# danisotelo/qm_door

Measured on AMD Instinct MI355X. Metric: MPC+WBC cycles/sec (AlienGo+Z1, N=100), higher is better.
Workload: dtype f64

## Files before the change

### qm_door_amd/csrc/kernels/aux_kernels.h

```cpp
#pragma once
#include "layout.h"
#include "lq_kernel.h"

namespace qmk {

__global__ void __launch_bounds__(64) input_weight_kernel(const ProblemR* P, const real* zeros, real* Rw) {
  __shared__ real J[12 * 12];
  __shared__ real RJ[12 * 12];
  const int lane = threadIdx.x;
  const ModelR& md = P->model;
  const int dd = lane < AD_DIRS ? lane : AD_DIRS - 1;
  const AdIn in{P->settings.initial_state, zeros, P->settings.initial_state, dd, 0.0_r};
  FlowOut<Du, Du3, Du3> f;
  BaseMotion2<Du, Du3> bm;
  centroidalSweep2<Du, Du3, Du3>(
      md, P->settings.gravity, in,
      [&](int c, Vec3<Du>, Vec3<Du3> v) {
        if (lane >= 3 && lane < 15) { const int j = lane - 3; J[(3 * c + 0) * 12 + j] = v.x.e; J[(3 * c + 1) * 12 + j] = v.y.e; J[(3 * c + 2) * 12 + j] = v.z.e; }
      },
      [&](Vec3<Du>, const Mat3<Du>&) { return Vec3<Du3>(); }, f, bm);
  __syncthreads();
  const real* Rt = P->settings.R_task;
  for (int e = lane; e < 144; e += 64) {
    const int i = e / 12, j = e % 12;
    real s = 0.0_r;
    for (int k = 0; k < 12; ++k) s += Rt[(12 + i) * 30 + 12 + k] * J[k * 12 + j];
    RJ[e] = s;
  }
  __syncthreads();
  for (int e = lane; e < 900; e += 64) {
    const int i = e / 30, j = e % 30;
    real v = Rt[e];
    if (i >= 12 && i < 24 && j >= 12 && j < 24) {
      v = 0.0_r;
// ... 102 lines not shown
      const real len = tb[q] - ta[q];
      const real a = (len > 2.0_r * REAL_EPS) ? (tb[q] - t[q]) / len : 1.0_r;
      const bool before = interval < 0 || K <= 1, after = !before && interval >= last;
      idx[q] = before ? 0 : (after ? max(last - 1, 0) : interval);
      alpha[q] = before ? 1.0_r : (after ? 0.0_r : a);
    }
    const bool isX = lane < 30, isU = lane >= 32 && lane < 62;
    const int c = isX ? lane : (isU ? lane - 32 : 0);
    real l[NB], r[NB];
#pragma unroll
    for (int q = 0; q < NB; ++q) {
      const int iu0 = min(idx[q], Np - 1), iu1 = min(idx[q] + 1, Np - 1);
      const real* pl = isU ? Up + (size_t(inst) * Np + iu0) * 30 : Xp + (size_t(inst) * (Np + 1) + idx[q]) * 30;
      const real* pr = isU ? Up + (size_t(inst) * Np + iu1) * 30 : Xp + (size_t(inst) * (Np + 1) + min(idx[q] + 1, last)) * 30;
      l[q] = pl[c]; r[q] = pr[c];
    }
    const real x0v = (x0 && isX) ? x0[size_t(inst) * 30 + c] : 0.0_r;
#pragma unroll
    for (int q = 0; q < NB; ++q) { QM_KEEP(l[q]); QM_KEEP(r[q]); }
#pragma unroll
    for (int q = 0; q < NB; ++q) {
      const int k = k0 + q;
      const real v = alpha[q] * l[q] + (1.0_r - alpha[q]) * r[q];
      if (k <= Nn && isX) warmX[(size_t(inst) * (Nn + 1) + k) * 30 + c] = (k == 0 && x0) ? x0v : v;
      else if (k < Nn && isU) warmU[(size_t(inst) * Nn + k) * 30 + c] = v;
    }
  }
}

__global__ void __launch_bounds__(64) policy_eval_kernel(int batch, int N, const real* tgrid, const real* X, const real* U, const int* modes, const real* tEval,
                                                         real* xOut, real* uOut, int* modeOut) {
  const int inst = blockIdx.x, lane = threadIdx.x;
  if (inst >= batch) return;
  const real* tg = tgrid + size_t(inst) * (N + 1);
  const real t = tEval[inst];
  int idx; real alpha;
  timeSegmentWave(tg, N + 1, t, lane, idx, alpha);
  const int kMode = gridCountBelow(tg + 1, N, t, lane);
  if (lane < 30) {
    const real* xl = X + (size_t(inst) * (N + 1) + idx) * 30;
    xOut[size_t(inst) * 30 + lane] = alpha * xl[lane] + (1.0_r - alpha) * xl[30 + lane];
  } else if (lane >= 32 && lane < 62) {
    const int i = lane - 32, iu0 = min(idx, N - 1), iu1 = min(idx + 1, N - 1);
    const real* ul = U + (size_t(inst) * N + iu0) * 30; const real* ur = U + (size_t(inst) * N + iu1) * 30;
    uOut[size_t(inst) * 30 + i] = alpha * ul[i] + (1.0_r - alpha) * ur[i];
  } else if (lane == 63) {
    modeOut[inst] = modes[size_t(inst) * (N + 1) + kMode];
  }
}

}
```

### qm_door_amd/csrc/kernels/gpu_rt.h

```cpp
#pragma once
#ifdef QMGPU_HOST_EMULATION
#include "real.h"
#include "simt_emu.h"
#else
#include <hip/hip_runtime.h>
#include "real.h"
namespace qmk {
#ifdef QM_WAVE_SYNC_BARE
#define QM_WAVE_SYNC() __builtin_amdgcn_wave_barrier()
#else
#define QM_WAVE_SYNC() do { __builtin_amdgcn_fence(__ATOMIC_RELEASE, "wavefront"); __builtin_amdgcn_wave_barrier(); __builtin_amdgcn_fence(__ATOMIC_ACQUIRE, "wavefront"); } while (0)
#endif
__device__ __forceinline__ double qmFromWords(int lo, int hi, double) { return __hiloint2double(hi, lo); }
__device__ __forceinline__ float qmFromWords(int lo, int, float) { return __int_as_float(lo); }
__device__ __forceinline__ int qmLoWord(double v) { return __double2loint(v); }
__device__ __forceinline__ int qmHiWord(double v) { return __double2hiint(v); }
__device__ __forceinline__ int qmLoWord(float v) { return __float_as_int(v); }
__device__ __forceinline__ int qmHiWord(float) { return 0; }
__device__ __forceinline__ real qmShflXor(real v, int mask) { return __shfl_xor(v, mask, 64); }
__device__ __forceinline__ real qmReadLane(real v, int src) {
  const int lo = __builtin_amdgcn_readlane(qmLoWord(v), src);
  const int hi = sizeof(real) == 8 ? __builtin_amdgcn_readlane(qmHiWord(v), src) : 0;
  return qmFromWords(lo, hi, real());
}
__device__ __forceinline__ int qmReadLaneInt(int v, int src) { return __builtin_amdgcn_readlane(v, src); }
__device__ __forceinline__ unsigned long long qmBallot(bool p) { return __builtin_amdgcn_ballot_w64(p); }
__device__ __forceinline__ int qmFirstBit(unsigned long long m) { return __builtin_ctzll(m); }
__device__ __forceinline__ int qmPopCount(unsigned long long m) { return __builtin_popcountll(m); }
typedef double QmAccD __attribute__((ext_vector_type(4)));
typedef float QmAccF __attribute__((ext_vector_type(4)));
template <class T> struct QmAccOf { typedef QmAccD type; };
template <> struct QmAccOf<float> { typedef QmAccF type; };
typedef QmAccOf<real>::type QmAcc;
typedef real QmD2 __attribute__((ext_vector_type(2)));
__device__ __forceinline__ void qmMfma(QmAccD& c, double a, double b) { c = __builtin_amdgcn_mfma_f64_16x16x4f64(a, b, c, 0, 0, 0); }
__device__ __forceinline__ void qmMfma(QmAccF& c, float a, float b) { c = __builtin_amdgcn_mfma_f32_16x16x4f32(a, b, c, 0, 0, 0); }
__device__ __forceinline__ constexpr int qmARow(int p) { return sizeof(real) == 8 ? p : (p >> 2) + 4 * (p & 3); }
__device__ __forceinline__ double qmMulNoFma(double a, double b) { return __dmul_rn(a, b); }
__device__ __forceinline__ double qmSubNoFma(double a, double b) { return __dsub_rn(a, b); }
__device__ __forceinline__ double qmRsqrtPos(double x) {
  const double y = __builtin_amdgcn_rsq(x);
  const double e = __builtin_fma(-x * y, y, 1.0);
  return __builtin_fma(y * e, __builtin_fma(e, 0.375, 0.5), y);
}
__device__ __forceinline__ float qmRsqrtPos(float x) { return __builtin_amdgcn_rsqf(x); }
__device__ __forceinline__ double qmRcpPos(double x) {
  double y = __builtin_amdgcn_rcp(x);
  y = __builtin_fma(y, __builtin_fma(-x, y, 1.0), y);
  return __builtin_fma(y, __builtin_fma(-x, y, 1.0), y);
}
__device__ __forceinline__ float qmRcpPos(float x) { return __builtin_amdgcn_rcpf(x); }
template <int R, bool FIRST> __device__ __forceinline__ void qmFmacRowBcast(double& acc, double bc, double m) {
  if (FIRST) asm volatile("s_nop 1\n\tv_fmac_f64_dpp %0, %1, %2 row_newbcast:%3 row_mask:0xf bank_mask:0xf" : "+v"(acc) : "v"(bc), "v"(m), "n"(R));
  else asm volatile("v_fmac_f64_dpp %0, %1, %2 row_newbcast:%3 row_mask:0xf bank_mask:0xf" : "+v"(acc) : "v"(bc), "v"(m), "n"(R));
}
template <int R, bool FIRST> __device__ __forceinline__ void qmFmacRowBcast(float& acc, float bc, float m) {
  if (FIRST) asm volatile("s_nop 1\n\tv_fmac_f32_dpp %0, %1, %2 row_newbcast:%3 row_mask:0xf bank_mask:0xf" : "+v"(acc) : "v"(bc), "v"(m), "n"(R));
  else asm volatile("v_fmac_f32_dpp %0, %1, %2 row_newbcast:%3 row_mask:0xf bank_mask:0xf" : "+v"(acc) : "v"(bc), "v"(m), "n"(R));
}
template <int G> __device__ __forceinline__ real qmReplicateRow(real v) {
  const int addr = (16 * G + (int(threadIdx.x) & 15)) * 4;
  const int lo = __builtin_amdgcn_ds_bpermute(addr, qmLoWord(v));
  const int hi = sizeof(real) == 8 ? __builtin_amdgcn_ds_bpermute(addr, qmHiWord(v)) : 0;
  return qmFromWords(lo, hi, real());
}
__device__ __forceinline__ real qmReplicateRow0(real v) { return qmReplicateRow<0>(v); }
#define QM_TO_LDS_PTR(T, p) ((const T __attribute__((address_space(3)))*)(p))
template <class T> __device__ __forceinline__ const T* qmConstantPtr(const T* p) {
  const T __attribute__((address_space(4)))* p4 = (const T __attribute__((address_space(4)))*)(p);
  asm("" : "+s"(p4));
  return (const T*)p4;
}
// ... 62 lines not shown
```

### qm_door_amd/csrc/kernels/linesearch_kernel.h

```cpp
#pragma once
#include "layout.h"
#include "ls_lds.h"
#include "schedule_dev.h"
#include "sweep_dev.h"

namespace qmk {

struct LsArgs {
  const ProblemR* P;
  const real* Rw;
  int batch, N, K, lineSearch;
  const real* eeContact;
  const real* tgrid; const real* dtgrid; const int* nodePhase;
  const real* X; const real* U; const real* dX; const real* dU;
  const real* targetTimes; const real* targetStates;
  const int* schedNum; const real* schedTimes; const int* schedModes;
  const real* metrics;
  const real* instStats;
  const int* nodeMode;
  real* Xt; real* Ut;
  real* outT; real* outX; real* outU; int* outMode; real* outStats;
  int iteration;
  int trialInLds;
  int* done;
};

inline int lsThreads(int B, int N, int cus) { return (B > cus && N + 1 <= LS_MAX_THREADS / 2) ? LS_MAX_THREADS / 2 : LS_MAX_THREADS; }
struct LsLaunch { int threads, dynamicLdsBytes, trialInLds; };
inline LsLaunch lsLaunch(int B, int N, int cus) {
  const int threads = lsThreads(B, N, cus), bytes = lsTrialLdsBytes(N, threads);
  return LsLaunch{threads, bytes, bytes > 0};
}

struct DblIn {
  const real* x; const real* u; real dtS; const real* k1;
  __device__ __forceinline__ real hn(int i) const { return x[i] + dtS * k1[i]; }
  __device__ __forceinline__ real euler(int i) const { return x[9 + i] + dtS * k1[9 + i]; }
  __device__ __forceinline__ real q(int j) const { return x[12 + j] + dtS * u[12 + j]; }
  __device__ __forceinline__ real qd(int j) const { return u[12 + j]; }
  __device__ __forceinline__ Vec3<real> force(int c) const { return Vec3<real>(u[3 * c], u[3 * c + 1], u[3 * c + 2]); }
};

template <class WP> __device__ __attribute__((noinline)) void nodePerformance(const ModelR& md, const SettingsR& st, WP Qw, WP Rw, int weightStructure, const real* bc, const Schedule& sched, const real* tTimes, const real* tStates, const real* contact, int K, real t, real dt, int phase,
                                       bool terminal, const real* x, const real* u, const real* xnext, real& cost, real& dyn, real& eq, real* xnOut = nullptr) {
  QM_TICK_DECL;
  const int mode = sched.modes[phase];
  real eePosRef[3], eeQuatRef[4];
  eeReference(tTimes, tStates, K, t, eePosRef, eeQuatRef);
  real Ke = 0.0_r, fRef[3] = {0.0_r, 0.0_r, 0.0_r}, pEnv[3] = {0.0_r, 0.0_r, 0.0_r};
  if (contact && !terminal) { Ke = st.ee_contact_stiffness; eeContactReference(tTimes, contact, K, t, fRef, pEnv); }
  real k1[12];
#pragma unroll
  for (int i = 0; i < 12; ++i) k1[i] = 0.0_r;
  real c = 0.0_r;
  dyn = 0.0_r; eq = 0.0_r;
  real phi[12];
#pragma unroll 1
// ... 110 lines not shown
}
__device__ __forceinline__ real sumSquaresStrided(const real* v, int n, int first, int stride) {
  constexpr int UN = 8;
  real s = 0.0_r;
  for (int base = first; base < n; base += UN * stride) {
    real t[UN];
#pragma unroll
    for (int q = 0; q < UN; ++q) { const int e = base + q * stride; t[q] = v[e < n ? e : first]; }
#pragma unroll
    for (int q = 0; q < UN; ++q) QM_KEEP(t[q]);
#pragma unroll
    for (int q = 0; q < UN; ++q) { const int e = base + q * stride; if (e < n) s += t[q] * t[q]; }
  }
  return s;
}

#ifdef QM_RICCATI_TIMING
#define QM_LS_CLOCK(slot) do { const unsigned long long n_ = clock64(); if (blockIdx.x == 0 && threadIdx.x == 0) qmk::qmRiccatiTicks[240 + (slot)] += n_ - lsClk; lsClk = n_; } while (0)
#else
#define QM_LS_CLOCK(slot)
#endif
#if defined(QM_LS_EXTERN) && !defined(QM_RICCATI_TIMING)
__global__ void __launch_bounds__(LS_MAX_THREADS) linesearch_kernel(LsArgs a);
#else
__global__ void __launch_bounds__(LS_MAX_THREADS) linesearch_kernel(LsArgs a) {
#ifdef QM_RICCATI_TIMING
  unsigned long long lsClk = clock64();
#endif
  __shared__ LsRed red; __shared__ LsCtlWords ctl; __shared__ LsVotes structVotes; __shared__ ModelR mdS;
  __shared__ __attribute__((aligned(16))) LsWeights wQ, wR;
  static_assert(lsLdsBytes(sizeof(red)) + lsLdsBytes(sizeof(ctl)) + lsLdsBytes(sizeof(structVotes)) + lsLdsBytes(sizeof(mdS)) + lsLdsBytes(sizeof(wQ)) + lsLdsBytes(sizeof(wR)) == LS_STATIC_LDS_BYTES,
                "a __shared__ array added here goes into this sum and into LS_STATIC_LDS_BYTES by hand: compare both with .group_segment_fixed_size in the assembly");
  const int inst = blockIdx.x, tid = threadIdx.x, nthr = blockDim.x;
  if (a.done[inst]) return;
  const int N = a.N;
  const SettingsR& st = a.P->settings;
  const real* tg = a.tgrid + size_t(inst) * (N + 1);
  const Schedule sched{a.schedNum[inst], a.schedTimes + size_t(inst) * QMGPU_MAX_EVENTS, a.schedModes + size_t(inst) * (QMGPU_MAX_EVENTS + 1)};
  const real* tTimes = a.targetTimes + size_t(inst) * a.K;
  const real* tStates = a.targetStates + size_t(inst) * a.K * QMGPU_NTARGET;
  const real* X = a.X + size_t(inst) * (N + 1) * 30; const real* U = a.U + size_t(inst) * N * 30;
  const real* dX = a.dX + size_t(inst) * (N + 1) * 30; const real* dU = a.dU + size_t(inst) * N * 30;
  const int half = (N + 1 <= nthr / 2) ? nthr / 2 : nthr;
  const int nTr = nthr / half, myTr = tid / half, ltid = tid - myTr * half;
  QM_DYNAMIC_LDS(trialLds);
  real* Xt = a.trialInLds ? trialLds + size_t(myTr) * lsTrialRows(N) * NX : a.Xt + (size_t(inst) * 2 + myTr) * (N + 1) * 30;
  real* Ut = a.trialInLds ? Xt + (N + 1) * NX : a.Ut + (size_t(inst) * 2 + myTr) * N * 30;

  constexpr int MDW = (int(sizeof(ModelR) / 4) + LS_MAX_THREADS - 1) / LS_MAX_THREADS;
  int mdw[2 * MDW];
  const int mdPer = nthr >= LS_MAX_THREADS ? MDW : 2 * MDW;
  real m0 = 0.0_r, d0 = 0.0_r, e0 = 0.0_r;
  {
    bool outside = false;
    real qv[4], rv4[4];
#pragma unroll
    for (int q4 = 0; q4 < 4; ++q4) { const int e = tid + q4 * nthr, ec = e < 900 ? e : tid; qv[q4] = st.Q[ec]; rv4[q4] = a.Rw[ec]; }
    {
      const int* src = reinterpret_cast<const int*>(&a.P->model);
#pragma unroll
      for (int w = 0; w < 2 * MDW; ++w) { const int e = tid + w * nthr; mdw[w] = (w < mdPer && e < int(sizeof(ModelR) / 4)) ? src[e] : 0; }
    }
    real mk[3] = {0.0_r, 0.0_r, 0.0_r};
    if (tid <= N) { const real* m = a.metrics + (size_t(inst) * (N + 1) + tid) * NODE_METRICS; mk[0] = m[0]; mk[1] = m[1]; mk[2] = m[2]; }
#pragma unroll
    for (int q4 = 0; q4 < 4; ++q4) { QM_KEEP(qv[q4]); QM_KEEP(rv4[q4]); }
#pragma unroll
    for (int w = 0; w < 2 * MDW; ++w) QM_KEEP(mdw[w]);
// ... 69 lines not shown
        const real al = tr ? alpha * st.alpha_decay : alpha;
        if (tr && al < st.alpha_min) break;
        real s0 = 0, s1 = 0, s2 = 0;
        const int nTrial = N + 1 < half ? N + 1 : half;
        for (int i = tr * half; i < tr * half + nTrial; ++i) { s0 += red[0][i]; s1 += red[1][i]; s2 += red[2][i]; }
        m1 = s0; v1 = sqrt(s1 + s2);
        bool ok;
        if (!a.lineSearch) { ok = true; type = 0; }
        else if (v1 > st.g_max) { ok = v1 < (1.0_r - st.gamma_c) * viol0; type = 1; }
        else if (v1 < st.g_min && viol0 < st.g_min && al * armijo < 0.0_r) { ok = m1 < merit0 + st.armijo_factor * al * armijo; type = 3; }
        else { ok = m1 < merit0 - st.gamma_c * viol0 || v1 < (1.0_r - st.gamma_c) * viol0; type = 2; }
        accAlpha = al;
        if (ok) acc = 1.0_r;
      }
      ctl[LS_MERIT1] = m1; ctl[LS_VIOL1] = v1; ctl[LS_ACCEPTED] = acc; ctl[LS_STEP_TYPE] = real(type); ctl[LS_ALPHA] = accAlpha;
    }
    __syncthreads();
    QM_LS_CLOCK(4);
    merit1 = ctl[LS_MERIT1]; viol1 = ctl[LS_VIOL1]; stepType = int(ctl[LS_STEP_TYPE]);
    accepted = ctl[LS_ACCEPTED] != 0.0_r;
    const real lastAlpha = ctl[LS_ALPHA];
    __syncthreads();
    if (accepted) { alpha = lastAlpha; break; }
    alpha = lastAlpha * st.alpha_decay;
    if (alpha < st.alpha_min) break;
  }
  if (!accepted) { alpha = 0.0_r; stepType = 4; merit1 = merit0; viol1 = viol0; }
  real* oX = a.outX + size_t(inst) * (N + 1) * 30; real* oU = a.outU + size_t(inst) * N * 30;
  axpyStrided(oX, X, dX, alpha, (N + 1) * 30, tid, nthr);
  axpyStrided(oU, U, dU, alpha, N * 30, tid, nthr);
  for (int k = tid; k <= N; k += nthr) { a.outT[size_t(inst) * (N + 1) + k] = tg[k]; a.outMode[size_t(inst) * (N + 1) + k] = a.nodeMode[size_t(inst) * (N + 1) + k]; }
  QM_LS_CLOCK(5);
  const real sx = sumSquaresStrided(dX, (N + 1) * 30, tid, nthr), su = sumSquaresStrided(dU, N * 30, tid, nthr);
  __syncthreads();
  red[0][tid] = sx; red[1][tid] = su;
  __syncthreads();
  if (tid == 0) {
    real s0 = 0, s1 = 0;
    for (int i = 0; i < nthr; ++i) { s0 += red[0][i]; s1 += red[1][i]; }
    int conv = 0;
    if (a.iteration + 1 >= st.sqp_iterations) conv = 1;
    else if (alpha < st.alpha_min) conv = 2;
    else if (fabs(merit1 - merit0) < st.cost_tol && viol1 < st.g_min) conv = 3;
    else if (alpha * sqrt(s0) < st.delta_tol && alpha * sqrt(s1) < st.delta_tol) conv = 4;
    if (ricStatus != 0.0_r && conv == 0) conv = 2;
    a.done[inst] = conv;
    if (a.outStats) {
      real* s = a.outStats + size_t(inst) * QMGPU_NSTATS;
      s[0] = merit0; s[1] = viol0; s[2] = merit1; s[3] = viol1; s[4] = alpha; s[5] = real(stepType); s[6] = armijo; s[7] = ricStatus;
      s[8] = real(a.iteration + 1); s[9] = real(conv);
    }
  }
  QM_LS_CLOCK(6);
}
#endif

}
```

### qm_door_amd/csrc/kernels/mpc_pipeline.h

```cpp
#pragma once
#include <vector>

#include "../host/host_error.h"
#include "aux_kernels.h"
#include "ddp_kernel.h"
#include "gpu_rt.h"
#include "layout.h"
#include "linesearch_kernel.h"
#include "lq_kernel.h"
#include "riccati_kernel.h"

namespace qmk {

struct MpcBuffers {
  ProblemR* dP = nullptr;
  real *dRw = nullptr, *dZeros = nullptr;
  real *dTgrid = nullptr, *dDtgrid = nullptr, *dX = nullptr, *dU = nullptr, *dStages = nullptr, *dAdRows = nullptr, *dMetrics = nullptr, *dGains = nullptr, *ddX = nullptr, *ddU = nullptr;
  real *dXt = nullptr, *dUt = nullptr, *dInstStats = nullptr, *dDebug = nullptr;
  int *dStageNc = nullptr, *dNodeMode = nullptr, *dNodePhase = nullptr, *dDone = nullptr;
  real *dDdpX = nullptr, *dDdpU = nullptr, *dDdpMerit = nullptr;
  int cus = 256;
  size_t maxBatch = 0, maxNodes = 0;
};

struct MpcIo {
  int batch, N, K, lineSearch;
  double dtD;
  const double *t0D, *timeGridD, *schedTimesD;
  const real *x0, *targetTimes, *targetStates;
  const int* schedNum; const real* schedTimes; const int* schedModes;
  const real *warmX, *warmU;
  real *outT, *outX, *outU; int* outMode; real* outStats;
  const real* eeContact;
  int algorithm;
};

template <class Alloc> inline void allocateMpcBuffers(MpcBuffers& m, size_t B, size_t N, Alloc&& alloc) {
  const size_t N1 = N + 1;
  m.maxBatch = B; m.maxNodes = N;
  auto R = [&](size_t n, bool scratch = true) { return static_cast<real*>(alloc(n, sizeof(real), scratch)); };
  auto I = [&](size_t n) { return static_cast<int*>(alloc(n, sizeof(int), true)); };
  m.dP = static_cast<ProblemR*>(alloc(1, sizeof(ProblemR), false));
  m.dRw = R(QM_RW_DOUBLES, false);
  m.dZeros = R(64, false);
  m.dTgrid = R(B * N1);
  m.dDtgrid = R(B * N1);
  m.dNodePhase = I(B * N1);
  m.dX = R(B * N1 * 30);
  m.dU = R(B * N * 30);
  m.dStages = R(B * N1 * STAGE_DOUBLES);
  m.dAdRows = R(B * N1 * AD_DOUBLES);
  m.dMetrics = R(B * N1 * NODE_METRICS);
  m.dGains = R(B * N * GAIN_DOUBLES);
  m.ddX = R(B * N1 * 30);
  m.ddU = R(B * N * 30);
  m.dXt = R(2 * B * N1 * 30);
  m.dUt = R(2 * B * N * 30);
  m.dInstStats = R(B * 4);
  m.dStageNc = I(B * N1);
  m.dNodeMode = I(B * N1);
  m.dDone = I(B);
  int dev = 0, cus = 0;
  if (hipGetDevice(&dev) == hipSuccess && hipDeviceGetAttribute(&cus, hipDeviceAttributeMultiprocessorCount, dev) == hipSuccess && cus > 0) m.cus = cus;
}

template <class Alloc> inline void ensureDdpBuffers(MpcBuffers& m, Alloc&& alloc) {
  if (m.dDdpX) return;
  const size_t B = m.maxBatch, N = m.maxNodes;
// ... 25 lines not shown
  io.warmX = in(a.warm_x, st.warmX, B * N1 * 30);
  io.warmU = in(a.warm_u, st.warmU, B * N * 30);
  io.eeContact = in(a.ee_contact_ref, st.eeContact, B * K * 6);
  io.outT = outT; io.outX = outX; io.outU = outU; io.outMode = a.out_mode; io.outStats = outStats;
  io.algorithm = a.algorithm;
  return io;
}

enum TimingEvent { EV_START, EV_AD_NODE, EV_LQ_NODE, EV_RICCATI, EV_LINE_SEARCH, EV_WBC_START, EV_WBC_END, TIMING_EVENTS = EV_WBC_END + 1 };
inline void recordTiming(hipEvent_t* ev, TimingEvent which, hipStream_t s) { if (ev) (void)hipEventRecord(ev[which], s); }

inline void enqueueLqRiccati(hipStream_t s, const MpcBuffers& m, const MpcIo& io, real* debug, hipEvent_t* ev) {
  const int B = io.batch, N = io.N;
  LqArgs la{m.dP, m.dRw, B, N, io.K, m.dTgrid, m.dDtgrid, m.dNodePhase, m.dX, m.dU, io.targetTimes, io.targetStates, io.schedNum, io.schedTimes,
            io.schedModes, m.dZeros, m.dStages, m.dStageNc, m.dNodeMode, m.dMetrics, debug, m.dAdRows, m.dDone, io.eeContact};
  QM_LAUNCH(ad_node_kernel, adGridFor(B * (N + 1)), 64, s, la);
  recordTiming(ev, EV_AD_NODE, s);
  QM_LAUNCH(lq_node_kernel, B * (N + 1), 64, s, la);
  recordTiming(ev, EV_LQ_NODE, s);
  RiccatiArgs ra{B, N, m.dStages, m.dStageNc, m.dDtgrid, io.x0, m.dX, m.dGains, m.ddX, m.ddU, m.dInstStats, m.dDone};
  QM_LAUNCH_DYN(riccati_kernel<RICCATI_WAVES>, B, RICCATI_WAVES * 64, RICCATI_LDS_BYTES, s, ra);
  recordTiming(ev, EV_RICCATI, s);
}

inline void enqueueMpcKernels(hipStream_t s, const MpcBuffers& m, const MpcIo& io, int iterations, bool debugLq, hipEvent_t* ev) {
  const int B = io.batch, N = io.N;
  recordTiming(ev, EV_START, s);
  for (int it = 0; it < iterations; ++it) {
    InitArgs ia{m.dP, B, N, io.dtD, io.t0D, io.timeGridD, io.schedTimesD, io.x0, it == 0 ? io.warmX : io.outX, it == 0 ? io.warmU : io.outU, io.schedNum, io.schedModes,
                m.dTgrid, m.dDtgrid, m.dNodePhase, m.dX, m.dU, it, m.dDone};
    QM_LAUNCH(mpc_init_kernel, B, 128, s, ia);
    enqueueLqRiccati(s, m, io, debugLq ? m.dDebug : nullptr, ev);
    const LsLaunch shape = lsLaunch(B, N, m.cus);
    LsArgs ls{m.dP, m.dRw, B, N, io.K, io.lineSearch, io.eeContact, m.dTgrid, m.dDtgrid, m.dNodePhase, m.dX, m.dU, m.ddX, m.ddU, io.targetTimes, io.targetStates, io.schedNum,
              io.schedTimes, io.schedModes, m.dMetrics, m.dInstStats, m.dNodeMode, m.dXt, m.dUt, io.outT, io.outX, io.outU, io.outMode, io.outStats, it, shape.trialInLds, m.dDone};
    QM_LAUNCH_DYN(linesearch_kernel, B, shape.threads, shape.dynamicLdsBytes, s, ls);
    recordTiming(ev, EV_LINE_SEARCH, s);
  }
}

inline void enqueueDdpKernels(hipStream_t s, const MpcBuffers& m, const MpcIo& io, int trials, hipEvent_t* ev) {
  const int B = io.batch, N = io.N;
  recordTiming(ev, EV_START, s);
  InitArgs ia{m.dP, B, N, io.dtD, io.t0D, io.timeGridD, io.schedTimesD, io.x0, io.warmX, io.warmU, io.schedNum, io.schedModes, m.dTgrid, m.dDtgrid, m.dNodePhase, m.dX, m.dU, 0, m.dDone};
  QM_LAUNCH(mpc_init_kernel, B, 128, s, ia);
  DdpArgs ra{m.dP, m.dRw, B, N, io.K, 0, io.eeContact, m.dTgrid, m.dDtgrid, m.dNodePhase, io.x0, m.dX, m.dU, io.targetTimes, io.targetStates, io.schedNum, io.schedTimes, io.schedModes,
             m.dStages, m.dStageNc, m.dGains, m.dX, m.dU, m.dDdpMerit};
  if (!io.warmX) QM_LAUNCH(ddp_rollout_kernel, (B + 63) / 64, 64, s, ra);
  enqueueLqRiccati(s, m, io, nullptr, ev);
  ra.trials = trials; ra.Xout = m.dDdpX; ra.Uout = m.dDdpU;
  QM_LAUNCH(ddp_rollout_kernel, (B * trials + 63) / 64, 64, s, ra);
  DdpSelectArgs sa{m.dP, B, N, trials, m.dTgrid, m.dNodeMode, m.dX, m.dU, m.dMetrics, m.dInstStats, m.dDdpX, m.dDdpU, m.dDdpMerit, io.outT, io.outX, io.outU, io.outMode, io.outStats, m.dDone};
  QM_LAUNCH(ddp_select_kernel, B, 256, s, sa);
  recordTiming(ev, EV_LINE_SEARCH, s);
}

inline int ddpTrialCount(double minStep, double maxStep) {
  int n = 0;
  for (double a = maxStep; a >= minStep && n < DDP_MAX_TRIALS; a *= 0.5) ++n;
  return n > 0 ? n : 1;
}

template <class Alloc> inline void enqueueMpcSolve(hipStream_t s, MpcBuffers& m, const MpcIo& io, const qmgpu_settings& settings, bool debugLq, hipEvent_t* ev, Alloc&& alloc) {
  if (io.algorithm != QMGPU_ALG_SQP && io.algorithm != QMGPU_ALG_DDP) throw std::invalid_argument("unknown qmgpu_mpc_args::algorithm");
  if (io.algorithm == QMGPU_ALG_DDP) {
    ensureDdpBuffers(m, alloc);
    enqueueDdpKernels(s, m, io, ddpTrialCount(settings.ddp_min_step, settings.ddp_max_step), ev);
  } else {
// ... 7 lines not shown
```

### qm_door_amd/csrc/qmgpu_api.hip

```cpp
#include <algorithm>
#include <cstdio>
#include <cstring>
#include <memory>
#include <string>
#include <vector>

#include "../../include/qmgpu.h"
#include "host/host_error.h"
#include "kernels/mpc_pipeline.h"
#include "kernels/feedback_kernel.h"
#include "kernels/value_kernel.h"
#include "kernels/dual_kernel.h"
#include "kernels/metrics_kernel.h"
#include "kernels/taskspace_kernel.h"
#include "kernels/wbc_kernel.h"
#include "kernels/frontend_kernel.h"
#include "kernels/plant_kernel.h"
#include "kernels/wbc_report_kernel.h"
#include "mpc32.h"

using namespace qmhost;
using namespace qmk;

struct DeviceGuard {
  int prev = -1;
  explicit DeviceGuard(int device, bool mayThrow = true) {
    if (hipGetDevice(&prev) != hipSuccess) prev = -1;
    if (prev == device) { prev = -1; return; }
    try { HIP_CHECK(hipSetDevice(device)); } catch (...) { prev = -1; if (mayThrow) throw; }
  }
  ~DeviceGuard() { if (prev >= 0) (void)hipSetDevice(prev); }
  DeviceGuard(const DeviceGuard&) = delete;
  DeviceGuard& operator=(const DeviceGuard&) = delete;
};

struct qmgpu_context {
  int device = 0, maxBatch = 0, maxNodes = 0;
  hipStream_t ownStream = nullptr, stream = nullptr;
  hipStream_t wbcStream = nullptr;
  hipEvent_t evPolicy = nullptr, evWbc = nullptr;
  bool overlap = false, wbcPending = false;
  qmgpu_problem hostProblem;
  int dtype = QMGPU_F64;
  MpcBuffers m;
  qmk32::Mpc32* m32 = nullptr;
  double *dPolX = nullptr, *dPolU = nullptr;
  int* dPolMode = nullptr;
  qmgpu_gait* dGaits = nullptr;
  std::vector<void*> allocations;
  bool timing = false, debugLq = false;
  static constexpr int kRing = 256;
  hipEvent_t ring[kRing][TIMING_EVENTS] = {};
  int ringKind[kRing];
  long callCount = 0;
  hipEvent_t* ev = ring[0];
  double lastMs[5] = {0, 0, 0, 0, 0};
  int lastBatch = 0, lastN = 0, lastAlgorithm = QMGPU_ALG_SQP;
  bool lastDebugLq = false;

  std::vector<std::pair<void*, size_t>> scratch;
  template <class T> T* alloc(size_t count, bool isScratch = true) {
    void* p = nullptr;
    HIP_CHECK(hipMalloc(&p, count * sizeof(T)));
    allocations.push_back(p);
    if (isScratch) scratch.emplace_back(p, count * sizeof(T));
    return static_cast<T*>(p);
  }
  const qmk32::RawAlloc rawAlloc = [this](size_t count, size_t elem, bool isScratch) { return static_cast<void*>(alloc<char>(count * elem, isScratch)); };

  qmgpu_context() = default;
  qmgpu_context(const qmgpu_context&) = delete;
  ~qmgpu_context() {
    DeviceGuard onDevice(device, false);
    if (ownStream) (void)hipStreamSynchronize(stream);
    if (wbcStream) { (void)hipStreamSynchronize(wbcStream); (void)hipStreamDestroy(wbcStream); }
    for (hipEvent_t e : {evPolicy, evWbc}) if (e) (void)hipEventDestroy(e);
    for (void* p : allocations) (void)hipFree(p);
    for (auto& set : ring) for (auto& e : set) if (e) (void)hipEventDestroy(e);
    if (ownStream) (void)hipStreamDestroy(ownStream);
    qmk32::destroy(m32);
// ... 10 lines not shown
  for (int l = 0; l < 4; ++l) ok = ok && m.parent[1 + 3 * l] == 0 && m.parent[2 + 3 * l] == 1 + 3 * l && m.parent[3 + 3 * l] == 2 + 3 * l;
  ok = ok && m.parent[13] == 0;
  for (int a = 1; a < 6; ++a) ok = ok && m.parent[13 + a] == 12 + a;
  bool seen[4] = {false, false, false, false};
  for (int c = 0; c < 4; ++c) { const int b = m.foot_body[c]; ok = ok && (b == 3 || b == 6 || b == 9 || b == 12); if (ok) seen[b / 3 - 1] = true; }
  ok = ok && seen[0] && seen[1] && seen[2] && seen[3] && m.ee_body == 18;
  for (int l = 0; l < 4; ++l) for (int j = 0; j < 3; ++j) ok = ok && m.axis[1 + 3 * l + j] == LEG_AXIS[j];
  for (int a = 0; a < 6; ++a) ok = ok && m.axis[13 + a] == ARM_AXIS[a];
  if (!ok) throw UnsupportedModel("kernels are specialised to the AlienGo+Z1 topology (4 x 3-joint legs + 6-joint arm)");
}

extern "C" {

int qmgpu_create(const qmgpu_problem* problem, int device, int max_batch, int max_nodes, qmgpu_handle* out) {
  return qmgpu_create_ex(problem, device, max_batch, max_nodes, QMGPU_F64, out);
}

int qmgpu_create_ex(const qmgpu_problem* problem, int device, int max_batch, int max_nodes, int dtype, qmgpu_handle* out) {
  if (!problem || !out || max_batch < 1 || max_nodes < 1 || (dtype != QMGPU_F64 && dtype != QMGPU_F32)) return setError(QMGPU_ERR_INVALID_ARGUMENT, "bad arguments to qmgpu_create");
  *out = nullptr;
  return guarded([&]() {
    checkTopology(problem->model);
    int count = 0;
    if (hipGetDeviceCount(&count) != hipSuccess || count <= 0) throw NoDevice("no HIP device visible; qm_door_amd has no CPU execution path");
    if (device < 0 || device >= count) throw NoDevice("HIP device index out of range");
    DeviceGuard onDevice(device);
    auto ctx = std::make_unique<qmgpu_context>();
    ctx->device = device; ctx->maxBatch = max_batch; ctx->maxNodes = max_nodes; ctx->hostProblem = *problem; ctx->dtype = dtype;
    HIP_CHECK(hipStreamCreate(&ctx->ownStream));
    ctx->stream = ctx->ownStream;
    const size_t B = size_t(max_batch), N = size_t(max_nodes);
    if (dtype == QMGPU_F64) allocateMpcBuffers(ctx->m, B, N, ctx->rawAlloc);
    else { ctx->m.dP = ctx->alloc<qmgpu_problem>(1, false); ctx->m.dRw = ctx->alloc<double>(qmk::QM_RW_DOUBLES, false); ctx->m.dZeros = ctx->alloc<double>(64, false); }
    ctx->dPolX = ctx->alloc<double>(B * 30);
    ctx->dPolU = ctx->alloc<double>(B * 30);
    ctx->dPolMode = ctx->alloc<int>(B);
    HIP_CHECK(hipMemcpy(ctx->m.dP, problem, sizeof(qmgpu_problem), hipMemcpyHostToDevice));
    HIP_CHECK(hipMemsetAsync(ctx->m.dZeros, 0, 64 * sizeof(double), ctx->stream));
    for (auto& set : ctx->ring) for (auto& e : set) HIP_CHECK(hipEventCreate(&e));
    HIP_CHECK(QM_ALLOW_DYNAMIC_LDS(wbc_kernel, WBC_LDS_BYTES));
    HIP_CHECK(prepareMpcKernels());
    HIP_CHECK(QM_ALLOW_DYNAMIC_LDS(value_function_kernel, VALUE_LDS_BYTES));
    HIP_CHECK(QM_ALLOW_DYNAMIC_LDS(metrics_kernel, METRICS_LDS_BYTES));
    HIP_CHECK(QM_ALLOW_DYNAMIC_LDS(taskspace_kernel, TASKSPACE_LDS_BYTES));
    QM_LAUNCH(input_weight_kernel, 1, 64, ctx->stream, ctx->m.dP, ctx->m.dZeros, ctx->m.dRw);
    HIP_CHECK(hipGetLastError());
    if (dtype == QMGPU_F32) ctx->m32 = qmk32::create(*problem, max_batch, max_nodes, ctx->stream, ctx->rawAlloc);
    HIP_CHECK(hipStreamSynchronize(ctx->stream));
    *out = ctx.release();
  });
}

int qmgpu_destroy(qmgpu_handle h) {
  delete h;
  return QMGPU_OK;
}

static void joinWbc(qmgpu_handle h) {
  if (h->wbcPending) { HIP_CHECK(hipStreamWaitEvent(h->stream, h->evWbc, 0)); h->wbcPending = false; }
}

int qmgpu_set_stream(qmgpu_handle h, void* hip_stream) {
  return onHandle(h, [&]() { h->stream = hip_stream ? static_cast<hipStream_t>(hip_stream) : h->ownStream; joinWbc(h); });
}

int qmgpu_synchronize(qmgpu_handle h) {
  return onHandle(h, [&]() { joinWbc(h); HIP_CHECK(hipStreamSynchronize(h->stream)); });
}

// ... 76 lines not shown
  return QMGPU_OK;
}
#endif

int qmgpu_debug_poison(qmgpu_handle h) {
  return onHandle(h, [&]() {
    joinWbc(h);
    for (auto& sc : h->scratch) HIP_CHECK(hipMemsetAsync(sc.first, 0xFF, sc.second, h->stream));
    constexpr int kDoubles = QM_CU_LDS_BYTES / 8;
    HIP_CHECK(QM_ALLOW_DYNAMIC_LDS(lds_poison_kernel, kDoubles * 8));
    QM_LAUNCH_DYN(lds_poison_kernel, 4096, 256, kDoubles * 8, h->stream, kDoubles, static_cast<double*>(nullptr));
    HIP_CHECK(hipGetLastError());
  });
}

int qmgpu_enable_debug(qmgpu_handle h, int enable) {
  return onHandle(h, [&]() {
    if (enable && h->dtype != QMGPU_F64) throw std::invalid_argument("the per-node LQ dump exists in the fp64 path only");
    if (enable && !h->m.dDebug) h->m.dDebug = h->alloc<double>(size_t(h->maxBatch) * (h->maxNodes + 1) * DBG_DOUBLES);
    h->debugLq = enable != 0;
  });
}

static void checkMpcArgs(qmgpu_handle h, const qmgpu_mpc_args* a) {
  if (!a) throw std::invalid_argument("null argument");
  if (a->batch < 1 || a->num_nodes < 1 || a->num_target_knots < 1) throw std::invalid_argument("batch, num_nodes and num_target_knots must be positive");
  if (a->batch > h->maxBatch || a->num_nodes > h->maxNodes) throw CapacityError("batch / num_nodes exceed the capacity given to qmgpu_create");
  if (h->dtype == QMGPU_F32 && a->num_target_knots > QMGPU_F32_MAX_TARGET_KNOTS) throw CapacityError("an fp32 handle stages at most QMGPU_F32_MAX_TARGET_KNOTS target knots per instance");
  if (!a->x0 || !a->target_times || !a->target_states || !a->sched_num_events || !a->sched_event_times || !a->sched_modes) throw std::invalid_argument("missing MPC input pointer");
  if (!a->time_grid && !a->t0) throw std::invalid_argument("either t0 or time_grid is required");
  if (!a->out_t || !a->out_x || !a->out_u || !a->out_mode) throw std::invalid_argument("missing MPC output pointer");
}

static void enqueueMpc(qmgpu_handle h, const qmgpu_mpc_args* a) {
  const qmgpu_settings& settings = h->hostProblem.settings;
  hipEvent_t* ev = h->timing ? h->ev : nullptr;
  if (h->dtype == QMGPU_F32) {
    qmk32::enqueue(h->m32, h->stream, a, settings, ev, h->rawAlloc);
  } else {
    const MpcIo io = makeMpcIo(*a, settings.dt, MpcStaging{}, [](const double* src, double*, size_t) { return src; }, a->out_t, a->out_x, a->out_u, a->out_stats);
    enqueueMpcSolve(h->stream, h->m, io, settings, h->debugLq, ev, h->rawAlloc);
  }
  h->lastBatch = a->batch; h->lastN = a->num_nodes; h->lastAlgorithm = a->algorithm;
  h->lastDebugLq = h->dtype == QMGPU_F64 && a->algorithm == QMGPU_ALG_SQP && h->debugLq;
}

static void enqueueWbc(qmgpu_handle h, const qmgpu_wbc_args* w, hipStream_t stream) {
  if (!w || w->batch < 1) throw std::invalid_argument("bad WBC arguments");
  if (w->batch > h->maxBatch) throw CapacityError("WBC batch exceeds the capacity given to qmgpu_create");
  if (!w->state_desired || !w->input_desired || !w->rbd_measured || !w->mode || !w->period || !w->time || !w->input_last || !w->out) throw std::invalid_argument("missing WBC pointer");
  static_assert(sizeof(unsigned long long) == sizeof(uint64_t), "working-set words");
  WbcArgs wa{h->m.dP, w->batch, w->variant, w->state_desired, w->input_desired, w->rbd_measured, w->mode, w->period, w->time, w->input_last, w->out, w->out_status, w->ee_force,
             reinterpret_cast<unsigned long long*>(w->working_set)};
  QM_LAUNCH_DYN(wbc_kernel, w->batch, WBC_THREADS, WBC_LDS_BYTES, stream, wa);
  HIP_CHECK(hipGetLastError());
}

static void beginTiming(qmgpu_handle h) {
  if (h->timing) h->ev = h->ring[h->callCount % qmgpu_context::kRing];
}
static void finishTiming(qmgpu_handle h, bool mpc, bool wbc, bool single = false) {
  if (!h->timing) return;
  h->ringKind[h->callCount % qmgpu_context::kRing] = (mpc ? 1 : 0) | (wbc ? 2 : 0) | (single ? 4 : 0);
  ++h->callCount;
}
static void readTiming(qmgpu_handle h, long call, double* ms6) {
  hipEvent_t* ev = h->ring[call % qmgpu_context::kRing];
  const int kind = h->ringKind[call % qmgpu_context::kRing];
  const bool mpc = kind & 1, wbc = kind & 2;
  if (kind & 4) {
    HIP_CHECK(hipEventSynchronize(ev[EV_LINE_SEARCH]));
    float ms = 0.f;
    HIP_CHECK(hipEventElapsedTime(&ms, ev[EV_START], ev[EV_LINE_SEARCH]));
    for (int i = 0; i < 6; ++i) ms6[i] = 0.0;
    ms6[5] = double(ms);
    return;
  }
// ... 173 lines not shown
  if (!a) return setError(QMGPU_ERR_INVALID_ARGUMENT, "null argument");
  return onHandle(h, [&]() {
    if (h->dtype != QMGPU_F64) throw std::invalid_argument("the WBC report exists for QMGPU_F64 handles only");
    if (a->batch < 1 || a->batch > h->maxBatch) throw std::invalid_argument("batch outside the capacity given to qmgpu_create");
    if (a->variant != 0 && a->variant != 1) throw std::invalid_argument("variant must be 0 (HierarchicalWbc) or 1 (HierarchicalMpcWbc)");
    if (a->x_stride != QMGPU_NWBC_DEC && a->x_stride != QMGPU_NWBC_OUT) throw std::invalid_argument("x_stride must be 36 or 54");
    if (!a->state_desired || !a->input_desired || !a->rbd_measured || !a->mode || !a->period || !a->time || !a->input_last || !a->x)
      throw std::invalid_argument("missing report pointer (state_desired, input_desired, rbd_measured, mode, period, time, input_last, x)");
    static_assert(sizeof(int) == sizeof(int32_t), "mode and rows words");
    qmwbcreport::ReportArgs ra{h->m.dP, a->batch, a->variant, a->x_stride, a->state_desired, a->input_desired, a->rbd_measured, a->mode, a->period, a->time, a->ee_force,
                               a->input_last, a->x, a->active_tol, a->eq_residual, a->ineq_margin, a->tau, a->rows, a->summary};
    QM_LAUNCH_DYN(qmwbcreport::wbc_report_kernel, a->batch, WBCREPORT_THREADS, WBCREPORT_LDS_BYTES, h->stream, ra);
    HIP_CHECK(hipGetLastError());
  });
}

int qmgpu_warm_start_batch(qmgpu_handle h, int batch, int prev_nodes, const double* prev_grid, const double* prev_X, const double* prev_U, int new_nodes,
                           const double* new_grid, const double* x0, double* warm_x, double* warm_u) {
  if (!prev_grid || !prev_X || !prev_U || !new_grid || !warm_x || !warm_u || batch < 1 || prev_nodes < 1 || new_nodes < 1)
    return setError(QMGPU_ERR_INVALID_ARGUMENT, "bad warm-start arguments");
  if (warm_x == prev_X || warm_u == prev_U) return setError(QMGPU_ERR_INVALID_ARGUMENT, "warm-start outputs must not alias the previous solution");
  return onHandle(h, [&]() {
    QM_LAUNCH(warm_start_kernel, batch, 256, h->stream, batch, prev_nodes, prev_grid, prev_X, prev_U, new_nodes, new_grid, x0, warm_x, warm_u);
    HIP_CHECK(hipGetLastError());
  });
}

int qmgpu_cycle_batch(qmgpu_handle h, const qmgpu_mpc_args* mpc, const double* t_eval, qmgpu_wbc_args* wbc) {
  if (!t_eval || !wbc) return setError(QMGPU_ERR_INVALID_ARGUMENT, "null argument");
  return onHandle(h, [&]() {
    checkMpcArgs(h, mpc);
    if (wbc->batch != mpc->batch) throw std::invalid_argument("MPC and WBC batch sizes differ");
    beginTiming(h);
    enqueueMpc(h, mpc);
    joinWbc(h);
    QM_LAUNCH(policy_eval_kernel, mpc->batch, 64, h->stream, mpc->batch, mpc->num_nodes, mpc->out_t, mpc->out_x, mpc->out_u, mpc->out_mode, t_eval, h->dPolX, h->dPolU,
              h->dPolMode);
    qmgpu_wbc_args w = *wbc;
    w.state_desired = h->dPolX; w.input_desired = h->dPolU; w.mode = h->dPolMode;
    hipStream_t ws = h->stream;
    if (h->overlap) {
      HIP_CHECK(hipEventRecord(h->evPolicy, h->stream));
      HIP_CHECK(hipStreamWaitEvent(h->wbcStream, h->evPolicy, 0));
      ws = h->wbcStream;
    }
    if (h->timing) HIP_CHECK(hipEventRecord(h->ev[EV_WBC_START], ws));
    enqueueWbc(h, &w, ws);
    if (h->timing) HIP_CHECK(hipEventRecord(h->ev[EV_WBC_END], ws));
    if (h->overlap) { HIP_CHECK(hipEventRecord(h->evWbc, ws)); h->wbcPending = true; }
    finishTiming(h, true, true);
  });
}

int qmgpu_debug_get_lq(qmgpu_handle h, int instance, int node, double* A, double* B, double* b, double* Q, double* R, double* q, double* r, double* C, double* D, double* e,
                       int32_t* nc) {
  return onHandle(h, [&]() {
    if (!h->debugLq || !h->m.dDebug) throw std::invalid_argument("call qmgpu_enable_debug(h, 1) before the solve");
    if (instance < 0 || instance >= h->lastBatch || node < 0 || node > h->lastN) throw std::invalid_argument("instance / node out of range");
    HIP_CHECK(hipStreamSynchronize(h->stream));
    std::vector<double> rec(DBG_DOUBLES);
    const size_t idx = size_t(instance) * (h->lastN + 1) + node;
    HIP_CHECK(hipMemcpy(rec.data(), h->m.dDebug + idx * DBG_DOUBLES, DBG_DOUBLES * sizeof(double), hipMemcpyDeviceToHost));
    int ncv = 0;
    HIP_CHECK(hipMemcpy(&ncv, h->m.dStageNc + idx, sizeof(int), hipMemcpyDeviceToHost));
    auto cp = [&](double* dst, int off, int n) { if (dst) std::memcpy(dst, rec.data() + off, n * sizeof(double)); };
    cp(A, DBG_A, 900); cp(B, DBG_B, 900); cp(b, DBG_b, 30); cp(Q, DBG_Q, 900); cp(R, DBG_R, 900); cp(q, DBG_q, 30); cp(r, DBG_r, 30);
    cp(C, DBG_C, 16 * 30); cp(D, DBG_D, 16 * 30); cp(e, DBG_e, 16);
    if (nc) *nc = ncv;
  });
}

int qmgpu_last_kernel_ms(qmgpu_handle h, double* ms6) {
  if (!ms6) return setError(QMGPU_ERR_INVALID_ARGUMENT, "null argument");
  return onHandle(h, [&]() {
    if (!h->timing || h->callCount == 0) throw std::invalid_argument("no timed call recorded (qmgpu_enable_timing)");
// ... 42 lines not shown
```

Baseline: 157,400.

## Fuse policy evaluation into the final line-search kernel epilogue

```diff
diff --git a/qm_door_amd/csrc/kernels/aux_kernels.h b/qm_door_amd/csrc/kernels/aux_kernels.h
--- a/qm_door_amd/csrc/kernels/aux_kernels.h
+++ b/qm_door_amd/csrc/kernels/aux_kernels.h
@@ -1,5 +1,30 @@
 #pragma once
 #include "layout.h"
+#include "schedule_dev.h"
+
+namespace qmk {
+
+__device__ __forceinline__ void policyEvalWave(int inst, int lane, int N, const real* tgrid, const real* X, const real* U, const int* modes, real t,
+                                               real* xOut, real* uOut, int* modeOut) {
+  const real* tg = tgrid + size_t(inst) * (N + 1);
+  int idx; real alpha;
+  timeSegmentWave(tg, N + 1, t, lane, idx, alpha);
+  const int kMode = gridCountBelow(tg + 1, N, t, lane);
+  if (lane < 30) {
+    const real* xl = X + (size_t(inst) * (N + 1) + idx) * 30;
+    xOut[size_t(inst) * 30 + lane] = qmLerp(alpha, xl[lane], xl[30 + lane]);
+  } else if (lane >= 32 && lane < 62) {
+    const int i = lane - 32, iu0 = min(idx, N - 1), iu1 = min(idx + 1, N - 1);
+    const real* ul = U + (size_t(inst) * N + iu0) * 30; const real* ur = U + (size_t(inst) * N + iu1) * 30;
+    uOut[size_t(inst) * 30 + i] = qmLerp(alpha, ul[i], ur[i]);
+  } else if (lane == 63) {
+    modeOut[inst] = modes[size_t(inst) * (N + 1) + kMode];
+  }
+}
+
+}
+
+#ifndef QM_LS_UNIT
 #include "lq_kernel.h"
 
 namespace qmk {
@@ -168,21 +193,8 @@
                                                          real* xOut, real* uOut, int* modeOut) {
   const int inst = blockIdx.x, lane = threadIdx.x;
   if (inst >= batch) return;
-  const real* tg = tgrid + size_t(inst) * (N + 1);
-  const real t = tEval[inst];
-  int idx; real alpha;
-  timeSegmentWave(tg, N + 1, t, lane, idx, alpha);
-  const int kMode = gridCountBelow(tg + 1, N, t, lane);
-  if (lane < 30) {
-    const real* xl = X + (size_t(inst) * (N + 1) + idx) * 30;
-    xOut[size_t(inst) * 30 + lane] = alpha * xl[lane] + (1.0_r - alpha) * xl[30 + lane];
-  } else if (lane >= 32 && lane < 62) {
-    const int i = lane - 32, iu0 = min(idx, N - 1), iu1 = min(idx + 1, N - 1);
-    const real* ul = U + (size_t(inst) * N + iu0) * 30; const real* ur = U + (size_t(inst) * N + iu1) * 30;
-    uOut[size_t(inst) * 30 + i] = alpha * ul[i] + (1.0_r - alpha) * ur[i];
-  } else if (lane == 63) {
-    modeOut[inst] = modes[size_t(inst) * (N + 1) + kMode];
-  }
-}
-
-}
+  policyEvalWave(inst, lane, N, tgrid, X, U, modes, tEval[inst], xOut, uOut, modeOut);
+}
+
+}
+#endif
diff --git a/qm_door_amd/csrc/kernels/gpu_rt.h b/qm_door_amd/csrc/kernels/gpu_rt.h
--- a/qm_door_amd/csrc/kernels/gpu_rt.h
+++ b/qm_door_amd/csrc/kernels/gpu_rt.h
@@ -1,7 +1,13 @@
 #pragma once
 #ifdef QMGPU_HOST_EMULATION
+#include <atomic>
 #include "real.h"
 #include "simt_emu.h"
+namespace qmk {
+inline real qmLerp(real alpha, real l, real r) { return alpha * l + (1.0_r - alpha) * r; }
+}
+#define QM_PUBLISH_STORES() std::atomic_thread_fence(std::memory_order_seq_cst)
+#define QM_ACQUIRE_STORES() std::atomic_thread_fence(std::memory_order_acquire)
 #else
 #include <hip/hip_runtime.h>
 #include "real.h"
@@ -38,6 +44,10 @@
 __device__ __forceinline__ constexpr int qmARow(int p) { return sizeof(real) == 8 ? p : (p >> 2) + 4 * (p & 3); }
 __device__ __forceinline__ double qmMulNoFma(double a, double b) { return __dmul_rn(a, b); }
 __device__ __forceinline__ double qmSubNoFma(double a, double b) { return __dsub_rn(a, b); }
+__device__ __forceinline__ double qmLerp(double alpha, double l, double r) { return __builtin_fma(alpha, l, __dmul_rn(1.0 - alpha, r)); }
+__device__ __forceinline__ float qmLerp(float alpha, float l, float r) { return __builtin_fmaf(alpha, l, __fmul_rn(1.0f - alpha, r)); }
+#define QM_PUBLISH_STORES() __threadfence()
+#define QM_ACQUIRE_STORES() __builtin_amdgcn_fence(__ATOMIC_ACQUIRE, "agent")
 __device__ __forceinline__ double qmRsqrtPos(double x) {
   const double y = __builtin_amdgcn_rsq(x);
   const double e = __builtin_fma(-x * y, y, 1.0);
diff --git a/qm_door_amd/csrc/kernels/linesearch_kernel.h b/qm_door_amd/csrc/kernels/linesearch_kernel.h
--- a/qm_door_amd/csrc/kernels/linesearch_kernel.h
+++ b/qm_door_amd/csrc/kernels/linesearch_kernel.h
@@ -3,6 +3,9 @@
 #include "ls_lds.h"
 #include "schedule_dev.h"
 #include "sweep_dev.h"
+#if !defined(QM_LS_EXTERN) || defined(QM_RICCATI_TIMING)
+#include "aux_kernels.h"
+#endif
 
 namespace qmk {
 
@@ -23,6 +26,7 @@
   int iteration;
   int trialInLds;
   int* done;
+  const real* tEval; real* polX; real* polU; int* polMode;
 };
 
 inline int lsThreads(int B, int N, int cus) { return (B > cus && N + 1 <= LS_MAX_THREADS / 2) ? LS_MAX_THREADS / 2 : LS_MAX_THREADS; }
@@ -199,8 +203,12 @@
   static_assert(lsLdsBytes(sizeof(red)) + lsLdsBytes(sizeof(ctl)) + lsLdsBytes(sizeof(structVotes)) + lsLdsBytes(sizeof(mdS)) + lsLdsBytes(sizeof(wQ)) + lsLdsBytes(sizeof(wR)) == LS_STATIC_LDS_BYTES,
                 "a __shared__ array added here goes into this sum and into LS_STATIC_LDS_BYTES by hand: compare both with .group_segment_fixed_size in the assembly");
   const int inst = blockIdx.x, tid = threadIdx.x, nthr = blockDim.x;
-  if (a.done[inst]) return;
   const int N = a.N;
+  const bool epilogue = sizeof(real) == 8 && a.polX != nullptr;
+  if (a.done[inst]) {
+    if (epilogue && tid < 64) policyEvalWave(inst, tid, N, a.outT, a.outX, a.outU, a.outMode, a.tEval[inst], a.polX, a.polU, a.polMode);
+    return;
+  }
   const SettingsR& st = a.P->settings;
   const real* tg = a.tgrid + size_t(inst) * (N + 1);
   const Schedule sched{a.schedNum[inst], a.schedTimes + size_t(inst) * QMGPU_MAX_EVENTS, a.schedModes + size_t(inst) * (QMGPU_MAX_EVENTS + 1)};
@@ -336,9 +344,14 @@
   for (int k = tid; k <= N; k += nthr) { a.outT[size_t(inst) * (N + 1) + k] = tg[k]; a.outMode[size_t(inst) * (N + 1) + k] = a.nodeMode[size_t(inst) * (N + 1) + k]; }
   QM_LS_CLOCK(5);
   const real sx = sumSquaresStrided(dX, (N + 1) * 30, tid, nthr), su = sumSquaresStrided(dU, N * 30, tid, nthr);
+  if (epilogue) QM_PUBLISH_STORES();
   __syncthreads();
   red[0][tid] = sx; red[1][tid] = su;
   __syncthreads();
+  if (epilogue && tid >= nthr - 64) {
+    QM_ACQUIRE_STORES();
+    policyEvalWave(inst, tid - (nthr - 64), N, a.outT, a.outX, a.outU, a.outMode, a.tEval[inst], a.polX, a.polU, a.polMode);
+  }
   if (tid == 0) {
     real s0 = 0, s1 = 0;
     for (int i = 0; i < nthr; ++i) { s0 += red[0][i]; s1 += red[1][i]; }
diff --git a/qm_door_amd/csrc/kernels/mpc_pipeline.h b/qm_door_amd/csrc/kernels/mpc_pipeline.h
--- a/qm_door_amd/csrc/kernels/mpc_pipeline.h
+++ b/qm_door_amd/csrc/kernels/mpc_pipeline.h
@@ -33,7 +33,9 @@
   real *outT, *outX, *outU; int* outMode; real* outStats;
   const real* eeContact;
   int algorithm;
+  const real* tEval; real *polX, *polU; int* polMode;
 };
+inline bool mpcRunsPolicyEpilogue(const MpcIo& io) { return sizeof(real) == 8 && io.algorithm == QMGPU_ALG_SQP && io.polX != nullptr; }
 
 template <class Alloc> inline void allocateMpcBuffers(MpcBuffers& m, size_t B, size_t N, Alloc&& alloc) {
   const size_t N1 = N + 1;
@@ -125,8 +127,10 @@
     QM_LAUNCH(mpc_init_kernel, B, 128, s, ia);
     enqueueLqRiccati(s, m, io, debugLq ? m.dDebug : nullptr, ev);
     const LsLaunch shape = lsLaunch(B, N, m.cus);
+    const bool pol = it == iterations - 1 && mpcRunsPolicyEpilogue(io);
     LsArgs ls{m.dP, m.dRw, B, N, io.K, io.lineSearch, io.eeContact, m.dTgrid, m.dDtgrid, m.dNodePhase, m.dX, m.dU, m.ddX, m.ddU, io.targetTimes, io.targetStates, io.schedNum,
-              io.schedTimes, io.schedModes, m.dMetrics, m.dInstStats, m.dNodeMode, m.dXt, m.dUt, io.outT, io.outX, io.outU, io.outMode, io.outStats, it, shape.trialInLds, m.dDone};
+              io.schedTimes, io.schedModes, m.dMetrics, m.dInstStats, m.dNodeMode, m.dXt, m.dUt, io.outT, io.outX, io.outU, io.outMode, io.outStats, it, shape.trialInLds, m.dDone,
+              pol ? io.tEval : nullptr, pol ? io.polX : nullptr, pol ? io.polU : nullptr, pol ? io.polMode : nullptr};
     QM_LAUNCH_DYN(linesearch_kernel, B, shape.threads, shape.dynamicLdsBytes, s, ls);
     recordTiming(ev, EV_LINE_SEARCH, s);
   }
diff --git a/qm_door_amd/csrc/qmgpu_api.hip b/qm_door_amd/csrc/qmgpu_api.hip
--- a/qm_door_amd/csrc/qmgpu_api.hip
+++ b/qm_door_amd/csrc/qmgpu_api.hip
@@ -44,8 +44,9 @@
   int dtype = QMGPU_F64;
   MpcBuffers m;
   qmk32::Mpc32* m32 = nullptr;
-  double *dPolX = nullptr, *dPolU = nullptr;
-  int* dPolMode = nullptr;
+  double *dPolX[2] = {nullptr, nullptr}, *dPolU[2] = {nullptr, nullptr};
+  int* dPolMode[2] = {nullptr, nullptr};
+  int polSet = 0;
   qmgpu_gait* dGaits = nullptr;
   std::vector<void*> allocations;
   bool timing = false, debugLq = false;
@@ -122,9 +123,11 @@
     const size_t B = size_t(max_batch), N = size_t(max_nodes);
     if (dtype == QMGPU_F64) allocateMpcBuffers(ctx->m, B, N, ctx->rawAlloc);
     else { ctx->m.dP = ctx->alloc<qmgpu_problem>(1, false); ctx->m.dRw = ctx->alloc<double>(qmk::QM_RW_DOUBLES, false); ctx->m.dZeros = ctx->alloc<double>(64, false); }
-    ctx->dPolX = ctx->alloc<double>(B * 30);
-    ctx->dPolU = ctx->alloc<double>(B * 30);
-    ctx->dPolMode = ctx->alloc<int>(B);
+    for (int set = 0; set < 2; ++set) {
+      ctx->dPolX[set] = ctx->alloc<double>(B * 30);
+      ctx->dPolU[set] = ctx->alloc<double>(B * 30);
+      ctx->dPolMode[set] = ctx->alloc<int>(B);
+    }
     HIP_CHECK(hipMemcpy(ctx->m.dP, problem, sizeof(qmgpu_problem), hipMemcpyHostToDevice));
     HIP_CHECK(hipMemsetAsync(ctx->m.dZeros, 0, 64 * sizeof(double), ctx->stream));
     for (auto& set : ctx->ring) for (auto& e : set) HIP_CHECK(hipEventCreate(&e));
@@ -267,17 +270,23 @@
   if (!a->out_t || !a->out_x || !a->out_u || !a->out_mode) throw std::invalid_argument("missing MPC output pointer");
 }
 
-static void enqueueMpc(qmgpu_handle h, const qmgpu_mpc_args* a) {
+struct PolicyOut { const double* tEval; double *x, *u; int* mode; };
+
+static bool enqueueMpc(qmgpu_handle h, const qmgpu_mpc_args* a, const PolicyOut* pol = nullptr) {
   const qmgpu_settings& settings = h->hostProblem.settings;
   hipEvent_t* ev = h->timing ? h->ev : nullptr;
+  bool evaluated = false;
   if (h->dtype == QMGPU_F32) {
     qmk32::enqueue(h->m32, h->stream, a, settings, ev, h->rawAlloc);
   } else {
-    const MpcIo io = makeMpcIo(*a, settings.dt, MpcStaging{}, [](const double* src, double*, size_t) { return src; }, a->out_t, a->out_x, a->out_u, a->out_stats);
+    MpcIo io = makeMpcIo(*a, settings.dt, MpcStaging{}, [](const double* src, double*, size_t) { return src; }, a->out_t, a->out_x, a->out_u, a->out_stats);
+    if (pol) { io.tEval = pol->tEval; io.polX = pol->x; io.polU = pol->u; io.polMode = pol->mode; }
+    evaluated = mpcRunsPolicyEpilogue(io);
     enqueueMpcSolve(h->stream, h->m, io, settings, h->debugLq, ev, h->rawAlloc);
   }
   h->lastBatch = a->batch; h->lastN = a->num_nodes; h->lastAlgorithm = a->algorithm;
   h->lastDebugLq = h->dtype == QMGPU_F64 && a->algorithm == QMGPU_ALG_SQP && h->debugLq;
+  return evaluated;
 }
 
 static void enqueueWbc(qmgpu_handle h, const qmgpu_wbc_args* w, hipStream_t stream) {
@@ -517,15 +526,17 @@
     checkMpcArgs(h, mpc);
     if (wbc->batch != mpc->batch) throw std::invalid_argument("MPC and WBC batch sizes differ");
     beginTiming(h);
-    enqueueMpc(h, mpc);
+    const int set = h->polSet ^ 1;
+    const PolicyOut pol{t_eval, h->dPolX[set], h->dPolU[set], h->dPolMode[set]};
+    if (!enqueueMpc(h, mpc, &pol))
+      QM_LAUNCH(policy_eval_kernel, mpc->batch, 64, h->stream, mpc->batch, mpc->num_nodes, mpc->out_t, mpc->out_x, mpc->out_u, mpc->out_mode, t_eval, pol.x, pol.u, pol.mode);
+    h->polSet = set;
+    qmgpu_wbc_args w = *wbc;
+    w.state_desired = pol.x; w.input_desired = pol.u; w.mode = pol.mode;
+    hipStream_t ws = h->stream;
+    if (h->overlap) HIP_CHECK(hipEventRecord(h->evPolicy, h->stream));
     joinWbc(h);
-    QM_LAUNCH(policy_eval_kernel, mpc->batch, 64, h->stream, mpc->batch, mpc->num_nodes, mpc->out_t, mpc->out_x, mpc->out_u, mpc->out_mode, t_eval, h->dPolX, h->dPolU,
-              h->dPolMode);
-    qmgpu_wbc_args w = *wbc;
-    w.state_desired = h->dPolX; w.input_desired = h->dPolU; w.mode = h->dPolMode;
-    hipStream_t ws = h->stream;
     if (h->overlap) {
-      HIP_CHECK(hipEventRecord(h->evPolicy, h->stream));
       HIP_CHECK(hipStreamWaitEvent(h->wbcStream, h->evPolicy, 0));
       ws = h->wbcStream;
     }
```

Result: slower. 155,700 (-1.1%).
